# unirestore/UniRestore

Hardware: AMD Instinct MI355X
Metric: restored 512x512 images/sec @ 20 denoise steps (whole job) (higher is better)
Workload: dtype bf16; 1 GPU; PIR 512x512 batch=8/GPU, 20 DDIM steps, bf16, hipGraph replay (BASELINE.json configs[1]; configs[2] shape for N=8); global_batch=8, per_gpu_batch=8, image=512, denoise_steps=20, parallelism=image-parallel dp1, weights=seeded random init (no checkpoints reachable)

## Files before the change

unirestore_amd/csrc/attention512.hip:

```cpp
#include "common.h"
#include "attention_params.h"

static __device__ uint4 g_attn512_zero_page[1];

namespace {

template <bool F16> struct Mfma32;
template <> struct Mfma32<false> {
  static __device__ __forceinline__ f32x4 run(const bf16x8& a, const bf16x8& b, const f32x4& c) { return __builtin_amdgcn_mfma_f32_16x16x32_bf16(a, b, c, 0, 0, 0); }
};
template <> struct Mfma32<true> {
  static __device__ __forceinline__ f32x4 run(const f16x8& a, const f16x8& b, const f32x4& c) { return __builtin_amdgcn_mfma_f32_16x16x32_f16(a, b, c, 0, 0, 0); }
};

constexpr int A5_D = 512, A5_BK = 64, A5_BQ = 32;
constexpr int A5_KT = A5_BK * A5_D * 2;
constexpr int A5_VT = A5_D * A5_BK * 2;
constexpr int A5_P = A5_BQ * 128;
constexpr int A5_LDS = A5_KT + A5_VT + A5_P + 4 * 32 * 4 + 32 * 4 + 4 * 32 * 4;

template <bool F16>
__global__ __launch_bounds__(256, 1) void attn512_kernel(const AttnP p) {
  constexpr int D = A5_D;
  typedef typename Frag<F16>::type frag_t;
  extern __shared__ __attribute__((aligned(16))) unsigned char smem[];
  unsigned char* ks = smem;
  unsigned char* vs = smem + A5_KT;
  unsigned char* ps = vs + A5_VT;
  float* smax = reinterpret_cast<float*>(ps + A5_P);
  float* salpha = smax + 128;
  float* ssum = salpha + 32;

  const int tid = threadIdx.x, lane = tid & 63, wid = tid >> 6;
  const int l15 = lane & 15, g4 = lane >> 4, l31 = lane & 31, hf = lane >> 5;
  const int bh = blockIdx.y, b = bh / p.H, h = bh - b * p.H;
  const int q0 = blockIdx.x * A5_BQ;
  const uint16_t* Q = p.q + b * p.bs_q + h * D;
  const uint16_t* K = p.k + b * p.bs_k + h * D;
  const uint16_t* V = p.vt + b * p.bs_vt + (long long)h * D * p.ldvt;

  frag_t qf[2][16];
#pragma unroll
  for (int qb = 0; qb < 2; ++qb) {
    const int qi = min(q0 + qb * 16 + l15, p.Tq - 1);
    const uint16_t* qp = Q + (long long)qi * p.ldq + g4 * 8;
#pragma unroll
    for (int ds = 0; ds < 16; ++ds) qf[qb][ds] = *reinterpret_cast<const frag_t*>(qp + ds * 32);
  }

  typedef __attribute__((address_space(1))) const void* gptr_t;
  typedef __attribute__((address_space(3))) void* lptr_t;
  const uint16_t* zero = reinterpret_cast<const uint16_t*>(g_attn512_zero_page);
  auto issue_k = [&](int kv0) {
#pragma unroll
    for (int i = 0; i < 16; ++i) {
      const int row = wid * 16 + i;
      const int chunk = lane ^ (row & 15);
      const uint16_t* g = kv0 + row < p.Tk ? K + (long long)(kv0 + row) * p.ldk + chunk * 8 : zero;
      __builtin_amdgcn_global_load_lds((gptr_t)g, (lptr_t)(ks + row * 1024), 16, 0, 0);
    }
  };
  const int lr = lane >> 3, pslot = lane & 7;
  auto issue_v = [&](int kv0) {
#pragma unroll
    for (int i = 0; i < 16; ++i) {
      const int piece = wid + 4 * i, row = piece * 8 + lr;
      const int chunk = pslot ^ ((row >> 1) & 7);
      const uint16_t* g = kv0 + chunk * 8 < p.ldvt ? V + (long long)row * p.ldvt + kv0 + chunk * 8 : zero;
      __builtin_amdgcn_global_load_lds((gptr_t)g, (lptr_t)(vs + piece * 1024), 16, 0, 0);
    }
  };

  f32x16 oacc[4];
#pragma unroll
  for (int f = 0; f < 4; ++f)
#pragma unroll
    for (int e = 0; e < 16; ++e) oacc[f][e] = 0.f;
  float m_run[2] = {-1e30f, -1e30f}, l_part[2] = {0.f, 0.f};
  const float c = p.scale_log2e;

  const int ntiles = (p.Tk + A5_BK - 1) / A5_BK;
  issue_k(0);
  issue_v(0);
  asm volatile("s_waitcnt vmcnt(16)" ::: "memory");
  __builtin_amdgcn_s_barrier();
  for (int t = 0; t < ntiles; ++t) {
    const bool more = t + 1 < ntiles;
    f32x4 sacc[2];
#pragma unroll
    for (int qb = 0; qb < 2; ++qb)
#pragma unroll
      for (int e = 0; e < 4; ++e) sacc[qb][e] = 0.f;
    {
      const unsigned char* krow = ks + (wid * 16 + l15) * 1024;
#pragma unroll
      for (int ds = 0; ds < 16; ++ds) {
        const frag_t kf = *reinterpret_cast<const frag_t*>(krow + (((ds * 4 + g4) ^ l15) << 4));
        sacc[0] = Mfma32<F16>::run(kf, qf[0][ds], sacc[0]);
        sacc[1] = Mfma32<F16>::run(kf, qf[1][ds], sacc[1]);
      }
    }
    if ((t + 1) * A5_BK > p.Tk) {
#pragma unroll
      for (int e = 0; e < 4; ++e)
        if (t * A5_BK + wid * 16 + g4 * 4 + e >= p.Tk) { sacc[0][e] = -INFINITY; sacc[1][e] = -INFINITY; }
    }
    float mx[2];
#pragma unroll
    for (int qb = 0; qb < 2; ++qb) {
      float m = fmaxf(fmaxf(sacc[qb][0], sacc[qb][1]), fmaxf(sacc[qb][2], sacc[qb][3]));
      m = fmaxf(m, __shfl_xor(m, 16, 64));
      m = fmaxf(m, __shfl_xor(m, 32, 64));
      mx[qb] = m;
    }
    if (g4 == 0) { smax[wid * 32 + l15] = mx[0]; smax[wid * 32 + 16 + l15] = mx[1]; }
    asm volatile("s_waitcnt lgkmcnt(0)" ::: "memory");
    __builtin_amdgcn_s_barrier();
    if (more) issue_k((t + 1) * A5_BK);
    float pr[2][4], alpha[2];
#pragma unroll
    for (int qb = 0; qb < 2; ++qb) {
      const int q = qb * 16 + l15;
      const float tm = fmaxf(fmaxf(smax[q], smax[32 + q]), fmaxf(smax[64 + q], smax[96 + q]));
      const float m_new = fmaxf(m_run[qb], tm);
      alpha[qb] = __builtin_amdgcn_exp2f((m_run[qb] - m_new) * c);
      m_run[qb] = m_new;
      const float mc = m_new * c;
      float sum = 0.f;
#pragma unroll
      for (int e = 0; e < 4; ++e) {
        pr[qb][e] = __builtin_amdgcn_exp2f(fmaf(sacc[qb][e], c, -mc));
        sum += pr[qb][e];
      }
      l_part[qb] = l_part[qb] * alpha[qb] + sum;
      const int slot = (2 * wid + (g4 >> 1)) ^ ((q >> 1) & 7);
      *reinterpret_cast<uint2*>(ps + q * 128 + (slot << 4) + ((g4 & 1) << 3)) =
          make_uint2(Act<F16>::pack2(pr[qb][0], pr[qb][1]), Act<F16>::pack2(pr[qb][2], pr[qb][3]));
    }
    if (wid == 0 && g4 == 0) { salpha[l15] = alpha[0]; salpha[16 + l15] = alpha[1]; }
    if (more) asm volatile("s_waitcnt vmcnt(16) lgkmcnt(0)" ::: "memory");
    else asm volatile("s_waitcnt vmcnt(0) lgkmcnt(0)" ::: "memory");
    __builtin_amdgcn_s_barrier();
    {
      const float a = salpha[l31];
      if (!__all(a == 1.f)) {
#pragma unroll
        for (int f = 0; f < 4; ++f)
#pragma unroll
          for (int e = 0; e < 16; ++e) oacc[f][e] *= a;
      }
#pragma unroll
      for (int kk = 0; kk < 4; ++kk) {
        const frag_t pf = *reinterpret_cast<const frag_t*>(ps + l31 * 128 + (((kk * 2 + hf) ^ ((l31 >> 1) & 7)) << 4));
#pragma unroll
        for (int f = 0; f < 4; ++f) {
          const int row = wid * 128 + f * 32 + l31;
          const frag_t vf = *reinterpret_cast<const frag_t*>(vs + row * 128 + (((kk * 2 + hf) ^ ((row >> 1) & 7)) << 4));
          oacc[f] = mfma16t(vf, pf, oacc[f]);
        }
      }
    }
    asm volatile("s_waitcnt vmcnt(0) lgkmcnt(0)" ::: "memory");
    __builtin_amdgcn_s_barrier();
    if (more) issue_v((t + 1) * A5_BK);
  }

#pragma unroll
  for (int qb = 0; qb < 2; ++qb) {
    float l = l_part[qb];
    l += __shfl_xor(l, 16, 64);
    l += __shfl_xor(l, 32, 64);
    if (g4 == 0) ssum[wid * 32 + qb * 16 + l15] = l;
  }
  asm volatile("s_waitcnt lgkmcnt(0)" ::: "memory");
  __builtin_amdgcn_s_barrier();
  const float inv = 1.f / (ssum[l31] + ssum[32 + l31] + ssum[64 + l31] + ssum[96 + l31]);
  const int qi = q0 + l31;
  if (qi < p.Tq) {
    uint16_t* op = p.o + b * p.bs_o + (long long)qi * p.ldo + h * D + wid * 128;
#pragma unroll
    for (int f = 0; f < 4; ++f)
#pragma unroll
      for (int g = 0; g < 4; ++g) {
        const int ch = f * 32 + 8 * g + 4 * hf;
        *reinterpret_cast<uint2*>(op + ch) =
            make_uint2(Act<F16>::pack2(oacc[f][g * 4] * inv, oacc[f][g * 4 + 1] * inv),
                       Act<F16>::pack2(oacc[f][g * 4 + 2] * inv, oacc[f][g * 4 + 3] * inv));
      }
  }
}

}

#ifndef UR_TU_F16
#define UR_TU_F16 0
#endif
#if UR_TU_F16
#define UR_ATTN512_LAUNCH ur_attn512_launch_f16
#else
#define UR_ATTN512_LAUNCH ur_attn512_launch_bf16
#endif

int UR_ATTN512_LAUNCH(const void* pp, hipStream_t s) {
  const AttnP& p = *static_cast<const AttnP*>(pp);
  constexpr bool F16 = UR_TU_F16 != 0;
  static ur::DeviceOnce attr_once;
  if (auto once_guard = attr_once.first()) {
    hipFuncSetAttribute(reinterpret_cast<const void*>(&attn512_kernel<F16>), hipFuncAttributeMaxDynamicSharedMemorySize, A5_LDS);
  }
  dim3 grid((p.Tq + A5_BQ - 1) / A5_BQ, p.B * p.H), block(256);
  hipLaunchKernelGGL((attn512_kernel<F16>), grid, block, A5_LDS, s, p);
  return ur::check_launch("ur_attention_fwd");
}
```

Baseline: 30.33 images/s.

## Share K/V tiles across two query groups in 512-thread attention blocks

Doubles the query tile per workgroup to 64 by running two 4-wave groups that share the same K/V LDS tiles, halving K/V global traffic per query. The block becomes 512 threads on a 1D grid, with an XCD-aware remap of block index to (batch, head, q-tile). It also software-pipelines the LDS fragment loads ahead of the MFMAs using sched_barrier, and adds a lazy max update with headroom so the rescale exp and accumulator rescale are skipped when the running max barely changes. The risks are higher register pressure and fewer workgroups per GPU, plus a small numerical difference from the lazy max.

```diff
diff --git a/unirestore_amd/csrc/attention512.hip b/unirestore_amd/csrc/attention512.hip
--- a/unirestore_amd/csrc/attention512.hip
+++ b/unirestore_amd/csrc/attention512.hip
@@ -13,28 +13,33 @@
   static __device__ __forceinline__ f32x4 run(const f16x8& a, const f16x8& b, const f32x4& c) { return __builtin_amdgcn_mfma_f32_16x16x32_f16(a, b, c, 0, 0, 0); }
 };
 
-constexpr int A5_D = 512, A5_BK = 64, A5_BQ = 32;
+constexpr int A5_D = 512, A5_BK = 64, A5_BQ = 64;
 constexpr int A5_KT = A5_BK * A5_D * 2;
 constexpr int A5_VT = A5_D * A5_BK * 2;
-constexpr int A5_P = A5_BQ * 128;
-constexpr int A5_LDS = A5_KT + A5_VT + A5_P + 4 * 32 * 4 + 32 * 4 + 4 * 32 * 4;
+constexpr int A5_P = 32 * 128;
+constexpr int A5_LDS = A5_KT + A5_VT + 2 * (A5_P + 4 * 32 * 4 + 32 * 4 + 4 * 32 * 4);
+constexpr float A5_HEADROOM = 8.f;
 
 template <bool F16>
-__global__ __launch_bounds__(256, 1) void attn512_kernel(const AttnP p) {
+__global__ __launch_bounds__(512) void attn512_kernel(const AttnP p) {
   constexpr int D = A5_D;
   typedef typename Frag<F16>::type frag_t;
   extern __shared__ __attribute__((aligned(16))) unsigned char smem[];
   unsigned char* ks = smem;
   unsigned char* vs = smem + A5_KT;
-  unsigned char* ps = vs + A5_VT;
-  float* smax = reinterpret_cast<float*>(ps + A5_P);
-  float* salpha = smax + 128;
-  float* ssum = salpha + 32;
-
-  const int tid = threadIdx.x, lane = tid & 63, wid = tid >> 6;
+  const int tid = threadIdx.x, lane = tid & 63;
+  const int wid = __builtin_amdgcn_readfirstlane(tid >> 6);
+  const int grp = wid >> 2, cw = wid & 3;
+  unsigned char* ps = vs + A5_VT + grp * A5_P;
+  float* smax = reinterpret_cast<float*>(vs + A5_VT + 2 * A5_P) + grp * 128;
+  float* salpha = reinterpret_cast<float*>(vs + A5_VT + 2 * A5_P) + 256 + grp * 32;
+  float* ssum = reinterpret_cast<float*>(vs + A5_VT + 2 * A5_P) + 320 + grp * 128;
+
   const int l15 = lane & 15, g4 = lane >> 4, l31 = lane & 31, hf = lane >> 5;
-  const int bh = blockIdx.y, b = bh / p.H, h = bh - b * p.H;
-  const int q0 = blockIdx.x * A5_BQ;
+  const int nq = (p.Tq + A5_BQ - 1) / A5_BQ, nwg = gridDim.x, wg = blockIdx.x;
+  const int item = (nwg & 7) == 0 ? (wg & 7) * (nwg >> 3) + (wg >> 3) : wg;
+  const int bh = item / nq, b = bh / p.H, h = bh - b * p.H;
+  const int q0 = (item - bh * nq) * A5_BQ + grp * 32;
   const uint16_t* Q = p.q + b * p.bs_q + h * D;
   const uint16_t* K = p.k + b * p.bs_k + h * D;
   const uint16_t* V = p.vt + b * p.bs_vt + (long long)h * D * p.ldvt;
@@ -51,23 +56,31 @@
   typedef __attribute__((address_space(1))) const void* gptr_t;
   typedef __attribute__((address_space(3))) void* lptr_t;
   const uint16_t* zero = reinterpret_cast<const uint16_t*>(g_attn512_zero_page);
-  auto issue_k = [&](int kv0) {
-#pragma unroll
-    for (int i = 0; i < 16; ++i) {
-      const int row = wid * 16 + i;
-      const int chunk = lane ^ (row & 15);
-      const uint16_t* g = kv0 + row < p.Tk ? K + (long long)(kv0 + row) * p.ldk + chunk * 8 : zero;
+  auto issue_k = [&](int kv0, int ln) {
+    const int kslot = ln ^ ((wid & 1) * 8);
+#pragma unroll
+    for (int i = 0; i < 8; ++i) {
+      const int row = wid * 8 + i;
+      const uint16_t* g = zero;
+      if (kv0 + row < p.Tk) g = K + (long long)(kv0 + row) * p.ldk + (kslot ^ i) * 8;
       __builtin_amdgcn_global_load_lds((gptr_t)g, (lptr_t)(ks + row * 1024), 16, 0, 0);
     }
   };
-  const int lr = lane >> 3, pslot = lane & 7;
-  auto issue_v = [&](int kv0) {
-#pragma unroll
-    for (int i = 0; i < 16; ++i) {
-      const int piece = wid + 4 * i, row = piece * 8 + lr;
-      const int chunk = pslot ^ ((row >> 1) & 7);
-      const uint16_t* g = kv0 + chunk * 8 < p.ldvt ? V + (long long)row * p.ldvt + kv0 + chunk * 8 : zero;
-      __builtin_amdgcn_global_load_lds((gptr_t)g, (lptr_t)(vs + piece * 1024), 16, 0, 0);
+  auto issue_v = [&](int kv0, int ln) {
+    const int vchunk = (ln & 7) ^ ((wid & 1) * 4 + (ln >> 4));
+    const long long vlane = (long long)(wid * 8 + (ln >> 3)) * p.ldvt + vchunk * 8;
+    const uint16_t* vb = V + kv0;
+    if (kv0 + A5_BK <= p.ldvt) {
+#pragma unroll
+      for (int i = 0; i < 8; ++i)
+        __builtin_amdgcn_global_load_lds((gptr_t)(vb + (long long)(64 * i) * p.ldvt + vlane), (lptr_t)(vs + (wid + 8 * i) * 1024), 16, 0, 0);
+    } else {
+      const bool ok = kv0 + vchunk * 8 < p.ldvt;
+#pragma unroll
+      for (int i = 0; i < 8; ++i) {
+        const uint16_t* g = ok ? vb + (long long)(64 * i) * p.ldvt + vlane : zero;
+        __builtin_amdgcn_global_load_lds((gptr_t)g, (lptr_t)(vs + (wid + 8 * i) * 1024), 16, 0, 0);
+      }
     }
   };
 
@@ -80,30 +93,46 @@
   const float c = p.scale_log2e;
 
   const int ntiles = (p.Tk + A5_BK - 1) / A5_BK;
-  issue_k(0);
-  issue_v(0);
-  asm volatile("s_waitcnt vmcnt(16)" ::: "memory");
+  issue_k(0, lane);
+  issue_v(0, lane);
+  asm volatile("s_waitcnt vmcnt(8)" ::: "memory");
   __builtin_amdgcn_s_barrier();
   for (int t = 0; t < ntiles; ++t) {
     const bool more = t + 1 < ntiles;
+    int ln = lane;
+    asm volatile("" : "+v"(ln));
+    const int l15 = ln & 15, g4 = ln >> 4, l31 = ln & 31, hf = ln >> 5;
     f32x4 sacc[2];
 #pragma unroll
     for (int qb = 0; qb < 2; ++qb)
 #pragma unroll
       for (int e = 0; e < 4; ++e) sacc[qb][e] = 0.f;
     {
-      const unsigned char* krow = ks + (wid * 16 + l15) * 1024;
-#pragma unroll
-      for (int ds = 0; ds < 16; ++ds) {
-        const frag_t kf = *reinterpret_cast<const frag_t*>(krow + (((ds * 4 + g4) ^ l15) << 4));
-        sacc[0] = Mfma32<F16>::run(kf, qf[0][ds], sacc[0]);
-        sacc[1] = Mfma32<F16>::run(kf, qf[1][ds], sacc[1]);
+      const unsigned char* krow = ks + (cw * 16 + l15) * 1024;
+      int kx = (g4 ^ l15) << 4;
+      asm volatile("" : "+v"(kx));
+      frag_t kf[2][2];
+#pragma unroll
+      for (int j = 0; j < 2; ++j) kf[0][j] = *reinterpret_cast<const frag_t*>(krow + (kx ^ (j << 6)));
+#pragma unroll
+      for (int dp = 0; dp < 8; ++dp) {
+        if (dp < 7) {
+#pragma unroll
+          for (int j = 0; j < 2; ++j) kf[(dp + 1) & 1][j] = *reinterpret_cast<const frag_t*>(krow + (kx ^ ((dp * 2 + 2 + j) << 6)));
+        }
+        __builtin_amdgcn_sched_barrier(0);
+#pragma unroll
+        for (int j = 0; j < 2; ++j) {
+          sacc[0] = Mfma32<F16>::run(kf[dp & 1][j], qf[0][dp * 2 + j], sacc[0]);
+          sacc[1] = Mfma32<F16>::run(kf[dp & 1][j], qf[1][dp * 2 + j], sacc[1]);
+        }
+        __builtin_amdgcn_sched_barrier(0);
       }
     }
     if ((t + 1) * A5_BK > p.Tk) {
 #pragma unroll
       for (int e = 0; e < 4; ++e)
-        if (t * A5_BK + wid * 16 + g4 * 4 + e >= p.Tk) { sacc[0][e] = -INFINITY; sacc[1][e] = -INFINITY; }
+        if (t * A5_BK + cw * 16 + g4 * 4 + e >= p.Tk) { sacc[0][e] = -INFINITY; sacc[1][e] = -INFINITY; }
     }
     float mx[2];
 #pragma unroll
@@ -113,17 +142,18 @@
       m = fmaxf(m, __shfl_xor(m, 32, 64));
       mx[qb] = m;
     }
-    if (g4 == 0) { smax[wid * 32 + l15] = mx[0]; smax[wid * 32 + 16 + l15] = mx[1]; }
+    if (g4 == 0) { smax[cw * 32 + l15] = mx[0]; smax[cw * 32 + 16 + l15] = mx[1]; }
     asm volatile("s_waitcnt lgkmcnt(0)" ::: "memory");
     __builtin_amdgcn_s_barrier();
-    if (more) issue_k((t + 1) * A5_BK);
+    if (more) issue_k((t + 1) * A5_BK, ln);
     float pr[2][4], alpha[2];
 #pragma unroll
     for (int qb = 0; qb < 2; ++qb) {
       const int q = qb * 16 + l15;
       const float tm = fmaxf(fmaxf(smax[q], smax[32 + q]), fmaxf(smax[64 + q], smax[96 + q]));
-      const float m_new = fmaxf(m_run[qb], tm);
-      alpha[qb] = __builtin_amdgcn_exp2f((m_run[qb] - m_new) * c);
+      const bool up = (tm - m_run[qb]) * c > A5_HEADROOM;
+      const float m_new = up ? tm : m_run[qb];
+      alpha[qb] = up ? __builtin_amdgcn_exp2f((m_run[qb] - m_new) * c) : 1.f;
       m_run[qb] = m_new;
       const float mc = m_new * c;
       float sum = 0.f;
@@ -133,12 +163,12 @@
         sum += pr[qb][e];
       }
       l_part[qb] = l_part[qb] * alpha[qb] + sum;
-      const int slot = (2 * wid + (g4 >> 1)) ^ ((q >> 1) & 7);
+      const int slot = (2 * cw + (g4 >> 1)) ^ ((q >> 1) & 7);
       *reinterpret_cast<uint2*>(ps + q * 128 + (slot << 4) + ((g4 & 1) << 3)) =
           make_uint2(Act<F16>::pack2(pr[qb][0], pr[qb][1]), Act<F16>::pack2(pr[qb][2], pr[qb][3]));
     }
-    if (wid == 0 && g4 == 0) { salpha[l15] = alpha[0]; salpha[16 + l15] = alpha[1]; }
-    if (more) asm volatile("s_waitcnt vmcnt(16) lgkmcnt(0)" ::: "memory");
+    if (cw == 0 && g4 == 0) { salpha[l15] = alpha[0]; salpha[16 + l15] = alpha[1]; }
+    if (more) asm volatile("s_waitcnt vmcnt(8) lgkmcnt(0)" ::: "memory");
     else asm volatile("s_waitcnt vmcnt(0) lgkmcnt(0)" ::: "memory");
     __builtin_amdgcn_s_barrier();
     {
@@ -149,20 +179,29 @@
 #pragma unroll
           for (int e = 0; e < 16; ++e) oacc[f][e] *= a;
       }
-#pragma unroll
-      for (int kk = 0; kk < 4; ++kk) {
-        const frag_t pf = *reinterpret_cast<const frag_t*>(ps + l31 * 128 + (((kk * 2 + hf) ^ ((l31 >> 1) & 7)) << 4));
-#pragma unroll
-        for (int f = 0; f < 4; ++f) {
-          const int row = wid * 128 + f * 32 + l31;
-          const frag_t vf = *reinterpret_cast<const frag_t*>(vs + row * 128 + (((kk * 2 + hf) ^ ((row >> 1) & 7)) << 4));
-          oacc[f] = mfma16t(vf, pf, oacc[f]);
+      int vx = (hf ^ ((l31 >> 1) & 7)) << 4;
+      asm volatile("" : "+v"(vx));
+      const unsigned char* prow = ps + l31 * 128;
+      const unsigned char* vrow = vs + (cw * 128 + l31) * 128;
+      frag_t pf[2], vf[3];
+      pf[0] = *reinterpret_cast<const frag_t*>(prow + vx);
+      vf[0] = *reinterpret_cast<const frag_t*>(vrow + vx);
+      vf[1] = *reinterpret_cast<const frag_t*>(vrow + 32 * 128 + vx);
+#pragma unroll
+      for (int i = 0; i < 16; ++i) {
+        if (i + 2 < 16) {
+          const int kk = (i + 2) >> 2, f = (i + 2) & 3;
+          if (f == 0) pf[kk & 1] = *reinterpret_cast<const frag_t*>(prow + (vx ^ (kk << 5)));
+          vf[(i + 2) % 3] = *reinterpret_cast<const frag_t*>(vrow + f * 32 * 128 + (vx ^ (kk << 5)));
         }
+        __builtin_amdgcn_sched_barrier(0);
+        oacc[i & 3] = mfma16t(vf[i % 3], pf[(i >> 2) & 1], oacc[i & 3]);
+        __builtin_amdgcn_sched_barrier(0);
       }
     }
     asm volatile("s_waitcnt vmcnt(0) lgkmcnt(0)" ::: "memory");
     __builtin_amdgcn_s_barrier();
-    if (more) issue_v((t + 1) * A5_BK);
+    if (more) issue_v((t + 1) * A5_BK, ln);
   }
 
 #pragma unroll
@@ -170,14 +209,14 @@
     float l = l_part[qb];
     l += __shfl_xor(l, 16, 64);
     l += __shfl_xor(l, 32, 64);
-    if (g4 == 0) ssum[wid * 32 + qb * 16 + l15] = l;
+    if (g4 == 0) ssum[cw * 32 + qb * 16 + l15] = l;
   }
   asm volatile("s_waitcnt lgkmcnt(0)" ::: "memory");
   __builtin_amdgcn_s_barrier();
   const float inv = 1.f / (ssum[l31] + ssum[32 + l31] + ssum[64 + l31] + ssum[96 + l31]);
   const int qi = q0 + l31;
   if (qi < p.Tq) {
-    uint16_t* op = p.o + b * p.bs_o + (long long)qi * p.ldo + h * D + wid * 128;
+    uint16_t* op = p.o + b * p.bs_o + (long long)qi * p.ldo + h * D + cw * 128;
 #pragma unroll
     for (int f = 0; f < 4; ++f)
 #pragma unroll
@@ -208,7 +247,7 @@
   if (auto once_guard = attr_once.first()) {
     hipFuncSetAttribute(reinterpret_cast<const void*>(&attn512_kernel<F16>), hipFuncAttributeMaxDynamicSharedMemorySize, A5_LDS);
   }
-  dim3 grid((p.Tq + A5_BQ - 1) / A5_BQ, p.B * p.H), block(256);
+  dim3 grid((p.Tq + A5_BQ - 1) / A5_BQ * p.B * p.H), block(512);
   hipLaunchKernelGGL((attn512_kernel<F16>), grid, block, A5_LDS, s, p);
   return ur::check_launch("ur_attention_fwd");
 }
```

After: 30.43 images/s, median of 6. About the same (+0.3%).
